# yisol/IDM-VTON

Hardware: NVIDIA H100
Metric: try-on images/sec @768x1024, 30 steps, CFG 2.0 (higher is better)
Workload: dtype fp16

## Files before the change

idm-vton_b200/csrc/attn.cu:

```cuda
#include <cuda_fp8.h>

#include <algorithm>

#include "common.cuh"
#include "host.h"
#include "wgmma.cuh"

namespace vton {

struct FlashParams {
  __half* out;
  int ld_out;
  int B, H, Nq, N0, N1;
  int D;
  int kv1_off;
  int kv1_count;
  const int* kv1_base;
  const int* kv1_rows;
  int causal;
  float scale_log2;
  int accumulate;
  float out_scale;
};

constexpr int FA_REGION = 128 * 128;
constexpr int FA_THREADS = 384;
constexpr int FA_PRODUCER_REGS = 40;
constexpr int FA_CONSUMER_REGS = 232;
constexpr uint32_t FA_BAR_TURN = 1;
constexpr uint32_t FA_BAR_CVT = 3;
constexpr int FA_CVT_THREADS = 96;

template <int R, bool KV8 = false>
struct FlashSmem {
  static constexpr int STAGES = R == 1 ? 3 : 2;
  static constexpr int OFF_Q = 0;
  static constexpr int OFF_K = OFF_Q + R * FA_REGION;
  static constexpr int OFF_V = OFF_K + STAGES * R * FA_REGION;
  static constexpr int STG_Q = 128 * 64;
  static constexpr int STG_BYTES = KV8 ? 2 * STG_Q + 2 * 128 : 0;
  static constexpr int OFF_STG = OFF_V + STAGES * R * FA_REGION;
  static constexpr int OFF_BAR = OFF_STG + STAGES * STG_BYTES;
  static constexpr int TOTAL = OFF_BAR + (KV8 ? 128 : 64) + 1024;
};

__device__ __forceinline__ float fast_exp2(float x) {
  float y;
  asm("ex2.approx.ftz.f32 %0, %1;" : "=f"(y) : "f"(x));
  return y;
}

__device__ __forceinline__ uint32_t kv8_scale_h2(int e) {
  const uint32_t hb = e >= -14 ? static_cast<uint32_t>(e + 15) << 10 : 1u << (e + 24);
  return hb | (hb << 16);
}
__device__ __forceinline__ uint32_t kv8_dequant2(uint32_t codes, uint32_t scale_h2) {
  const __half2_raw r = __nv_cvt_fp8x2_to_halfraw2(static_cast<__nv_fp8x2_storage_t>(codes & 0xffffu), __NV_E4M3);
  __half2 v(r);
  const __half2 s = *reinterpret_cast<const __half2*>(&scale_h2);
  v = __hmul2_rn(v, s);
  return *reinterpret_cast<uint32_t*>(&v);
}

template <int KS, bool IP, int R, int DN, bool KV8>
__device__ __forceinline__ void flash_body(const CUtensorMap* tmQ, const CUtensorMap* tmK0, const CUtensorMap* tmV0,
                                           const CUtensorMap* tmK1, const CUtensorMap* tmV1, const CUtensorMap* tmE,
                                           const FlashParams p) {
  static_assert(!KV8 || (KS == 4 && !IP && R == 1 && DN == 64), "the FP8 segment 1 is for D = 64 without IP");
  using SM = FlashSmem<R, KV8>;
  constexpr int ST = SM::STAGES;
  constexpr bool OVERLAP = DN == 64 && !IP;
  extern __shared__ uint8_t smem_raw[];
  const uint32_t smem_base = (smem_u32(smem_raw) + 1023u) & ~1023u;
  const uint32_t bar_base = smem_base + SM::OFF_BAR;
  const uint32_t q_full = bar_base;
  auto kv_full = [&](int s) { return bar_base + 8u * (1 + s); };
  auto kv_empty = [&](int s) { return bar_base + 8u * (1 + ST + s); };
  auto stg_full = [&](int s) { return bar_base + 8u * (1 + 2 * ST + s); };

  const int warp = threadIdx.x >> 5;
  const int lane = threadIdx.x & 31;
  const int wg = threadIdx.x >> 7;
  const int q_tile = blockIdx.x;
  const int h = blockIdx.y;
  int b = blockIdx.z;
  if (p.N1 > 0 && p.kv1_off > 0 && p.kv1_off < p.B) {
    b += p.kv1_off;
    if (b >= p.B) b -= p.B;
  }

  if (threadIdx.x == 0) {
    mbar_init(q_full, 1);
    for (int s = 0; s < ST; ++s) {
      mbar_init(kv_full(s), 1);
      mbar_init(kv_empty(s), 2);
      if constexpr (KV8) mbar_init(stg_full(s), 1);
    }
    fence_barrier_init();
  }
  if (threadIdx.x == 256) {
    tma_prefetch_desc(tmQ);
    tma_prefetch_desc(tmK0);
    tma_prefetch_desc(tmV0);
    if (p.N1 > 0) {
      tma_prefetch_desc(tmK1);
      tma_prefetch_desc(tmV1);
      if constexpr (KV8) tma_prefetch_desc(tmE);
    }
  }
  pdl_wait();
  __syncthreads();
  pdl_launch_dependents();

  const int tiles0 = (p.N0 + 127) >> 7;
  int idx1 = -1;
  if (p.N1 > 0) {
    idx1 = b - p.kv1_off;
    if (idx1 >= 0 && p.kv1_rows) {
      idx1 = p.kv1_rows[idx1];
      if (idx1 >= p.kv1_count) idx1 = -1;
    } else if (idx1 >= 0) {
      idx1 = idx1 % p.kv1_count + (p.kv1_base ? *p.kv1_base : 0);
    }
  }
  const bool zero_kv = (p.N1 > 0) && (idx1 < 0);
  const int tiles1 = (p.N1 > 0 && idx1 >= 0) ? ((p.N1 + 127) >> 7) : 0;
  const int total = p.causal ? min(tiles0, q_tile + 1) : tiles0 + tiles1;

  if (wg == 2) {
    setmaxnreg_dec<FA_PRODUCER_REGS>();
    if (threadIdx.x == 256) {
      mbar_expect_tx(q_full, R * FA_REGION);
#pragma unroll
      for (int r = 0; r < R; ++r)
        tma_load_3d(smem_base + SM::OFF_Q + r * FA_REGION, tmQ, q_full, h * p.D + r * 64, q_tile * 128, b);
      for (int j = 0; j < total; ++j) {
        const int stage = j % ST;
        if (j >= ST) mbar_wait(kv_empty(stage), ((j / ST) - 1) & 1);
        if constexpr (KV8) {
          if (j >= tiles0) {
            const uint32_t stg = smem_base + SM::OFF_STG + stage * SM::STG_BYTES;
            const int key0 = (j - tiles0) * 128;
            mbar_expect_tx(stg_full(stage), SM::STG_BYTES);
            tma_load_3d(stg, tmK1, stg_full(stage), h * 64, key0, idx1);
            tma_load_3d(stg + SM::STG_Q, tmV1, stg_full(stage), h * 64, key0, idx1);
            tma_load_3d(stg + 2 * SM::STG_Q, tmE, stg_full(stage), key0, h, idx1);
            tma_load_3d(stg + 2 * SM::STG_Q + 128, tmE, stg_full(stage), key0, p.H + h, idx1);
            continue;
          }
        }
        mbar_expect_tx(kv_full(stage), 2 * R * FA_REGION);
#pragma unroll
        for (int r = 0; r < R; ++r) {
          const uint32_t kdst = smem_base + SM::OFF_K + (stage * R + r) * FA_REGION;
          const uint32_t vdst = smem_base + SM::OFF_V + (stage * R + r) * FA_REGION;
          const int col = h * p.D + r * 64;
          if (j < tiles0) {
            tma_load_3d(kdst, tmK0, kv_full(stage), col, j * 128, b);
            tma_load_3d(vdst, tmV0, kv_full(stage), col, j * 128, b);
          } else {
            tma_load_3d(kdst, tmK1, kv_full(stage), col, (j - tiles0) * 128, idx1);
            tma_load_3d(vdst, tmV1, kv_full(stage), col, (j - tiles0) * 128, idx1);
          }
        }
      }
    } else if constexpr (KV8) {
      if (warp >= 9) {
        const int t = threadIdx.x - 288;
        for (int j = tiles0; j < total; ++j) {
          const int stage = j % ST;
          mbar_wait(stg_full(stage), ((j - tiles0) / ST) & 1);
          const uint32_t stg = smem_base + SM::OFF_STG + stage * SM::STG_BYTES;
#pragma unroll 1
          for (int c = t; c < 2 * 128 * 8; c += FA_CVT_THREADS) {
            const int kv = c >> 10, r = (c >> 3) & 127, ch = c & 7;
            uint32_t lo, hi;
            int e;
            asm volatile("ld.shared.v2.u32 {%0, %1}, [%2];" : "=r"(lo), "=r"(hi) : "r"(stg + kv * SM::STG_Q + r * 64 + ch * 8));
            asm volatile("ld.shared.s8 %0, [%1];" : "=r"(e) : "r"(stg + 2 * SM::STG_Q + kv * 128 + r));
            const uint32_t sc = kv8_scale_h2(e);
            const uint32_t dst = smem_base + (kv ? SM::OFF_V : SM::OFF_K) + stage * FA_REGION + r * 128 + ((ch ^ (r & 7)) << 4);
            asm volatile("st.shared.v4.u32 [%0], {%1, %2, %3, %4};" ::"r"(dst), "r"(kv8_dequant2(lo, sc)),
                         "r"(kv8_dequant2(lo >> 16, sc)), "r"(kv8_dequant2(hi, sc)), "r"(kv8_dequant2(hi >> 16, sc))
                         : "memory");
          }
          fence_proxy_async_smem();
          named_bar_sync(FA_BAR_CVT, FA_CVT_THREADS);
          if (t == 0) mbar_arrive(kv_full(stage));
        }
      }
    }
    return;
  }

  setmaxnreg_inc<FA_CONSUMER_REGS>();
  const int row0 = wg * 64 + ((warp & 3) << 4) + (lane >> 2);
  const int qi0 = q_tile * 128 + row0, qi1 = qi0 + 8;
  const int cq = (lane & 3) * 2;
  const float sl2 = p.scale_log2;
  float m0 = -INFINITY, m1 = -INFINITY, l0 = 0.f, l1 = 0.f;
  float o[DN / 2];
#pragma unroll
  for (int i = 0; i < DN / 2; ++i) o[i] = 0.f;
  uint32_t o_seg0[IP ? DN / 4 : 1];
#pragma unroll
  for (int i = 0; i < (IP ? DN / 4 : 1); ++i) o_seg0[i] = 0u;
  float s[64];
  uint32_t pa[8][4];

  const uint32_t q_src = smem_base + SM::OFF_Q + wg * (64 * 128);
  auto issue_s = [&](int stage) {
    const uint32_t k_src = smem_base + SM::OFF_K + stage * R * FA_REGION;
    wgmma_fence();
#pragma unroll
    for (int k = 0; k < KS; ++k) {
      const uint32_t off = (k >> 2) * FA_REGION + (k & 3) * 32;
      WgmmaF16SS<128, 0>::mma(s, make_gmma_desc_sw128(q_src + off, 0, 1024), make_gmma_desc_sw128(k_src + off, 0, 1024),
                              k > 0 ? 1 : 0);
    }
    wgmma_commit();
  };
  auto issue_pv = [&](int stage) {
    const uint32_t v_src = smem_base + SM::OFF_V + stage * R * FA_REGION;
    wgmma_fence();
#pragma unroll
    for (int kk = 0; kk < 8; ++kk)
      WgmmaF16RS<DN>::mma(o, pa[kk], make_gmma_desc_sw128(v_src + kk * 2048, FA_REGION, 1024), 1);
    wgmma_commit();
  };
  auto turn_begin = [&]() { named_bar_sync(FA_BAR_TURN + wg, 256); };
  auto turn_end = [&](bool last) {
    if (!(last && wg == 1)) named_bar_arrive(FA_BAR_TURN + (wg ^ 1), 256);
  };
  auto softmax = [&](int j, float& alpha0, float& alpha1) {
    const int key0 = (j < tiles0) ? j * 128 : (j - tiles0) * 128;
    const int kv_valid = (j < tiles0) ? min(128, p.N0 - key0) : min(128, p.N1 - key0);
    const bool masked = p.causal || kv_valid < 128;
    float mx0 = -INFINITY, mx1 = -INFINITY;
    if (masked) {
#pragma unroll
      for (int i = 0; i < 16; ++i) {
#pragma unroll
        for (int u = 0; u < 2; ++u) {
          const int col = i * 8 + cq + u;
          bool ok = col < kv_valid;
          const bool ok0 = ok && (!p.causal || key0 + col <= qi0);
          const bool ok1 = ok && (!p.causal || key0 + col <= qi1);
          if (!ok0) s[4 * i + u] = -INFINITY;
          if (!ok1) s[4 * i + 2 + u] = -INFINITY;
          mx0 = fmaxf(mx0, s[4 * i + u]);
          mx1 = fmaxf(mx1, s[4 * i + 2 + u]);
        }
      }
    } else {
#pragma unroll
      for (int i = 0; i < 16; ++i) {
#pragma unroll
        for (int u = 0; u < 2; ++u) {
          mx0 = fmaxf(mx0, s[4 * i + u]);
          mx1 = fmaxf(mx1, s[4 * i + 2 + u]);
        }
      }
    }
    mx0 = fmaxf(mx0, __shfl_xor_sync(0xffffffffu, mx0, 1));
    mx0 = fmaxf(mx0, __shfl_xor_sync(0xffffffffu, mx0, 2));
    mx1 = fmaxf(mx1, __shfl_xor_sync(0xffffffffu, mx1, 1));
    mx1 = fmaxf(mx1, __shfl_xor_sync(0xffffffffu, mx1, 2));
    const float mn0 = fmaxf(m0, mx0), mn1 = fmaxf(m1, mx1);
    alpha0 = fast_exp2((m0 - mn0) * sl2);
    alpha1 = fast_exp2((m1 - mn1) * sl2);
    const float ms0 = mn0 * sl2, ms1 = mn1 * sl2;
    m0 = mn0;
    m1 = mn1;
    float sum0 = 0.f, sum1 = 0.f;
    if (masked) {
#pragma unroll
      for (int i = 0; i < 16; ++i) {
#pragma unroll
        for (int u = 0; u < 2; ++u) {
          const float x0 = s[4 * i + u], x1 = s[4 * i + 2 + u];
          const float p0 = x0 == -INFINITY ? 0.f : fast_exp2(x0 * sl2 - ms0);
          const float p1 = x1 == -INFINITY ? 0.f : fast_exp2(x1 * sl2 - ms1);
          s[4 * i + u] = p0;
          s[4 * i + 2 + u] = p1;
          sum0 += p0;
          sum1 += p1;
        }
      }
    } else {
#pragma unroll
      for (int i = 0; i < 16; ++i) {
#pragma unroll
        for (int u = 0; u < 2; ++u) {
          const float p0 = fast_exp2(s[4 * i + u] * sl2 - ms0);
          const float p1 = fast_exp2(s[4 * i + 2 + u] * sl2 - ms1);
          s[4 * i + u] = p0;
          s[4 * i + 2 + u] = p1;
          sum0 += p0;
          sum1 += p1;
        }
      }
    }
    l0 = l0 * alpha0 + sum0;
    l1 = l1 * alpha1 + sum1;
  };
  auto pack_p = [&]() {
#pragma unroll
    for (int kk = 0; kk < 8; ++kk) {
      pa[kk][0] = pack_h2(s[8 * kk + 0], s[8 * kk + 1]);
      pa[kk][1] = pack_h2(s[8 * kk + 2], s[8 * kk + 3]);
      pa[kk][2] = pack_h2(s[8 * kk + 4], s[8 * kk + 5]);
      pa[kk][3] = pack_h2(s[8 * kk + 6], s[8 * kk + 7]);
    }
  };

  auto rescale_o = [&](float alpha0, float alpha1) {
#pragma unroll
    for (int i = 0; i < DN / 8; ++i) {
      o[4 * i] *= alpha0;
      o[4 * i + 1] *= alpha0;
      o[4 * i + 2] *= alpha1;
      o[4 * i + 3] *= alpha1;
    }
  };
  auto close_segment0 = [&](float ls0, float ls1) {
    ls0 += __shfl_xor_sync(0xffffffffu, ls0, 1);
    ls0 += __shfl_xor_sync(0xffffffffu, ls0, 2);
    ls1 += __shfl_xor_sync(0xffffffffu, ls1, 1);
    ls1 += __shfl_xor_sync(0xffffffffu, ls1, 2);
    const float i0 = 1.f / ls0, i1 = 1.f / ls1;
#pragma unroll
    for (int i = 0; i < DN / 8; ++i) {
      if constexpr (IP) {
        o_seg0[2 * i] = pack_h2(o[4 * i] * i0, o[4 * i + 1] * i0);
        o_seg0[2 * i + 1] = pack_h2(o[4 * i + 2] * i1, o[4 * i + 3] * i1);
      }
      o[4 * i] = o[4 * i + 1] = o[4 * i + 2] = o[4 * i + 3] = 0.f;
    }
  };

  if (wg == 1) named_bar_arrive(FA_BAR_TURN, 256);
  mbar_wait(q_full, 0);
  if constexpr (OVERLAP) {
    mbar_wait(kv_full(0), 0);
    turn_begin();
    issue_s(0);
    turn_end(false);
    wgmma_wait<0>();
    fence_regs(s);
    {
      float a0, a1;
      softmax(0, a0, a1);
    }
    pack_p();
    for (int j = 1; j < total; ++j) {
      const int stage = j % ST, prev = (j - 1) % ST;
      mbar_wait(kv_full(stage), (j / ST) & 1);
      turn_begin();
      issue_s(stage);
      issue_pv(prev);
      turn_end(false);
      wgmma_wait<1>();
      fence_regs(s);
      const bool seg_start = IP && j == tiles0;
      float ls0 = l0, ls1 = l1;
      if (seg_start) {
        m0 = m1 = -INFINITY;
        l0 = l1 = 0.f;
      }
      float alpha0, alpha1;
      softmax(j, alpha0, alpha1);
      wgmma_wait<0>();
      fence_regs(o);
      if ((threadIdx.x & 127) == 0) mbar_arrive(kv_empty(prev));
      if (seg_start)
        close_segment0(ls0, ls1);
      else
        rescale_o(alpha0, alpha1);
      pack_p();
    }
    turn_begin();
    issue_pv((total - 1) % ST);
    turn_end(true);
    wgmma_wait<0>();
    fence_regs(o);
  } else {
    for (int j = 0; j < total; ++j) {
      const int stage = j % ST;
      mbar_wait(kv_full(stage), (j / ST) & 1);
      turn_begin();
      issue_s(stage);
      turn_end(false);
      wgmma_wait<0>();
      fence_regs(s);
      const bool seg_start = IP && j == tiles0;
      float ls0 = l0, ls1 = l1;
      if (seg_start) {
        m0 = m1 = -INFINITY;
        l0 = l1 = 0.f;
      }
      float alpha0, alpha1;
      softmax(j, alpha0, alpha1);
      if (seg_start)
        close_segment0(ls0, ls1);
      else
        rescale_o(alpha0, alpha1);
      pack_p();
      fence_regs(o);
      turn_begin();
      issue_pv(stage);
      turn_end(j == total - 1);
      wgmma_wait<0>();
      fence_regs(o);
      if ((threadIdx.x & 127) == 0) mbar_arrive(kv_empty(stage));
    }
  }

  l0 += __shfl_xor_sync(0xffffffffu, l0, 1);
  l0 += __shfl_xor_sync(0xffffffffu, l0, 2);
  l1 += __shfl_xor_sync(0xffffffffu, l1, 1);
  l1 += __shfl_xor_sync(0xffffffffu, l1, 2);
  if (zero_kv) {
    const float mn0 = fmaxf(m0, 0.f), mn1 = fmaxf(m1, 0.f);
    const float alpha0 = fast_exp2((m0 - mn0) * sl2), alpha1 = fast_exp2((m1 - mn1) * sl2);
    l0 = l0 * alpha0 + static_cast<float>(p.N1) * fast_exp2(-mn0 * sl2);
    l1 = l1 * alpha1 + static_cast<float>(p.N1) * fast_exp2(-mn1 * sl2);
#pragma unroll
    for (int i = 0; i < DN / 8; ++i) {
      o[4 * i] *= alpha0;
      o[4 * i + 1] *= alpha0;
      o[4 * i + 2] *= alpha1;
      o[4 * i + 3] *= alpha1;
    }
  }
  const float inv[2] = {1.f / l0, 1.f / l1};
  const int qi[2] = {qi0, qi1};
  const bool two_softmax = IP && tiles1 > 0;
#pragma unroll
  for (int hr = 0; hr < 2; ++hr) {
    if (qi[hr] >= p.Nq) continue;
    __half* dst = p.out + (static_cast<long long>(b) * p.Nq + qi[hr]) * p.ld_out + h * p.D;
#pragma unroll
    for (int i = 0; i < DN / 8; ++i) {
      const int col = i * 8 + cq;
      if (col >= p.D) continue;
      float v0 = o[4 * i + 2 * hr] * inv[hr], v1 = o[4 * i + 2 * hr + 1] * inv[hr];
      if (two_softmax) {
        const float2 t = unpack_h2(o_seg0[IP ? 2 * i + hr : 0]);
        v0 = t.x + round_h(p.out_scale * round_h(v0));
        v1 = t.y + round_h(p.out_scale * round_h(v1));
      } else if (p.accumulate) {
        const float2 a = unpack_h2(*reinterpret_cast<const uint32_t*>(dst + col));
        v0 = a.x + round_h(p.out_scale * round_h(v0));
        v1 = a.y + round_h(p.out_scale * round_h(v1));
      }
      *reinterpret_cast<uint32_t*>(dst + col) = pack_h2(v0, v1);
    }
  }
}

template <int KS, bool IP = false, int R = (KS + 3) / 4, int DN = (KS <= 4 ? 64 : 96)>
__global__ void __launch_bounds__(FA_THREADS, 1)
flash_kernel(const __grid_constant__ CUtensorMap tmQ, const __grid_constant__ CUtensorMap tmK0,
             const __grid_constant__ CUtensorMap tmV0, const __grid_constant__ CUtensorMap tmK1,
             const __grid_constant__ CUtensorMap tmV1, const FlashParams p) {
  flash_body<KS, IP, R, DN, false>(&tmQ, &tmK0, &tmV0, &tmK1, &tmV1, nullptr, p);
}

__global__ void __launch_bounds__(FA_THREADS, 1)
flash_kv8_kernel(const __grid_constant__ CUtensorMap tmQ, const __grid_constant__ CUtensorMap tmK0,
                 const __grid_constant__ CUtensorMap tmV0, const __grid_constant__ CUtensorMap tmK1,
                 const __grid_constant__ CUtensorMap tmV1, const __grid_constant__ CUtensorMap tmE, const FlashParams p) {
  flash_body<4, false, 1, 64, true>(&tmQ, &tmK0, &tmV0, &tmK1, &tmV1, &tmE, p);
}

void set_attn_poly(int) {}
void set_attn_qtiles(int) {}
void set_attn_v2(int) {}

static int encode_tokens(CUtensorMap* tm, const void* base, long long ld, int cols, int n, int batch) {
  uint64_t dims[3] = {static_cast<uint64_t>(cols), static_cast<uint64_t>(n), static_cast<uint64_t>(batch)};
  uint64_t strides[2] = {static_cast<uint64_t>(ld) * 2, static_cast<uint64_t>(n) * ld * 2};
  uint32_t box[3] = {64, 128, 1};
  return encode_tmap_f16(tm, base, 3, dims, strides, box);
}

template <int KS, bool IP = false>
static int launch_flash(const CUtensorMap& tmQ, const CUtensorMap& tmK0, const CUtensorMap& tmV0, const CUtensorMap& tmK1,
                        const CUtensorMap& tmV1, const FlashParams& p, cudaStream_t stream) {
  constexpr int R = (KS + 3) / 4;
  auto kern = flash_kernel<KS, IP>;
  static bool configured = false;
  if (!configured) {
    VTON_CUDA(cudaFuncSetAttribute(kern, cudaFuncAttributeMaxDynamicSharedMemorySize, FlashSmem<R>::TOTAL));
    configured = true;
  }
  dim3 grid((p.Nq + 127) / 128, p.H, p.B);
  VTON_CUDA(launch_kernel(kern, grid, dim3(FA_THREADS), FlashSmem<R>::TOTAL, stream, tmQ, tmK0, tmV0, tmK1, tmV1, p));
  count_launch();
  return kOk;
}

static int flash(const void* q, long long ldq, const void* k0, const void* v0, long long ldkv0, const void* k1,
                 const void* v1, long long ldkv1, int B1, void* out, long long ldo, FlashParams p, cudaStream_t stream,
                 bool ip = false) {
  CUtensorMap tmQ, tmK0, tmV0, tmK1, tmV1;
  const int cols = p.H * p.D;
  if (int e = encode_tokens(&tmQ, q, ldq, cols, p.Nq, p.B)) return e;
  if (int e = encode_tokens(&tmK0, k0, ldkv0, cols, p.N0, p.B)) return e;
  if (int e = encode_tokens(&tmV0, v0, ldkv0, cols, p.N0, p.B)) return e;
  tmK1 = tmK0;
  tmV1 = tmV0;
  if (k1 != nullptr) {
    if (int e = encode_tokens(&tmK1, k1, ldkv1, cols, p.N1, B1)) return e;
    if (int e = encode_tokens(&tmV1, v1, ldkv1, cols, p.N1, B1)) return e;
  }
  p.out = static_cast<__half*>(out);
  p.ld_out = static_cast<int>(ldo);
  if (ip) return launch_flash<4, true>(tmQ, tmK0, tmV0, tmK1, tmV1, p, stream);
  switch (p.D / 16) {
    case 1: return launch_flash<1>(tmQ, tmK0, tmV0, tmK1, tmV1, p, stream);
    case 2: return launch_flash<2>(tmQ, tmK0, tmV0, tmK1, tmV1, p, stream);
    case 3: return launch_flash<3>(tmQ, tmK0, tmV0, tmK1, tmV1, p, stream);
    case 4: return launch_flash<4>(tmQ, tmK0, tmV0, tmK1, tmV1, p, stream);
    case 5: return launch_flash<5>(tmQ, tmK0, tmV0, tmK1, tmV1, p, stream);
    case 6: return launch_flash<6>(tmQ, tmK0, tmV0, tmK1, tmV1, p, stream);
  }
  set_last_error("attention: head dim %d unsupported", p.D);
  return kErrUnsupported;
}

static int attn_common(const void* q, long long ldq, const void* k0, const void* v0, long long ldkv0, const void* k1,
                       const void* v1, long long ldkv1, void* out, long long ldo, int B, int H, int Nq, int N0, int N1,
                       int B1, int kv1_off, int kv1_mod, const void* kv1_base, const void* kv1_rows, float scale,
                       int accumulate, cudaStream_t stream) {
  VTON_CHECK_ARG(B > 0 && H > 0 && Nq > 0 && N0 > 0 && N1 >= 0, "attn: bad sizes B=%d H=%d Nq=%d N0=%d N1=%d", B, H, Nq, N0, N1);
  VTON_CHECK_ARG(ldq % 8 == 0 && ldkv0 % 8 == 0 && ldo % 8 == 0, "attn: row strides must be multiples of 8");
  VTON_CHECK_ARG(aligned_to(out, 4), "attn: out must be 4-byte aligned (stored two halves at a time)");
  VTON_CHECK_ARG(B <= 65535 && H <= 65535, "attn: grid too large");
  const bool has1 = N1 > 0 && B1 > 0 && k1 && v1;
  VTON_CHECK_ARG(N1 == 0 || has1 || kv1_off >= B, "attn: segment 1 declared (N1=%d) but no K/V given", N1);
  VTON_CHECK_ARG(!has1 || ldkv1 % 8 == 0, "attn: ldkv1 must be a multiple of 8");
  FlashParams p{};
  p.B = B;
  p.H = H;
  p.Nq = Nq;
  p.N0 = N0;
  p.N1 = N1;
  p.D = 64;
  p.kv1_off = has1 ? kv1_off : (N1 > 0 ? B : 0);
  p.kv1_count = has1 ? (kv1_rows || kv1_mod <= 0 ? B1 : kv1_mod) : 1;
  p.kv1_base = has1 && !kv1_rows ? static_cast<const int*>(kv1_base) : nullptr;
  p.kv1_rows = has1 ? static_cast<const int*>(kv1_rows) : nullptr;
  p.scale_log2 = scale * 1.4426950408889634f;
  p.accumulate = accumulate;
  p.out_scale = 1.f;
  return flash(q, ldq, k0, v0, ldkv0, has1 ? k1 : nullptr, has1 ? v1 : nullptr, ldkv1, B1, out, ldo, p, stream);
}

int attn_impl(const void* q, long long ldq, const void* k0, const void* v0, long long ldkv0, const void* k1,
              const void* v1, long long ldkv1, void* out, long long ldo, int B, int H, int Nq, int N0, int N1, int B1,
              int kv1_off, int kv1_mod, const void* kv1_base, float scale, int accumulate, cudaStream_t stream) {
  return attn_common(q, ldq, k0, v0, ldkv0, k1, v1, ldkv1, out, ldo, B, H, Nq, N0, N1, B1, kv1_off, kv1_mod, kv1_base,
                     nullptr, scale, accumulate, stream);
}

int attn_rows_impl(const void* q, long long ldq, const void* k0, const void* v0, long long ldkv0, const void* k1,
                   const void* v1, long long ldkv1, void* out, long long ldo, int B, int H, int Nq, int N0, int N1,
                   int B1, int kv1_off, const void* kv1_rows, float scale, int accumulate, cudaStream_t stream) {
  VTON_CHECK_ARG(kv1_rows, "attention_rows: kv1_rows is null");
  VTON_CHECK_ARG(aligned_to(kv1_rows, 4), "attention_rows: kv1_rows must be 4-byte aligned (int32)");
  VTON_CHECK_ARG(N1 > 0 && B1 > 0 && k1 && v1, "attention_rows: needs segment-1 K/V (N1=%d, B1=%d)", N1, B1);
  VTON_CHECK_ARG(kv1_off >= 0 && kv1_off < B, "attention_rows: kv1_off %d outside [0, B=%d)", kv1_off, B);
  return attn_common(q, ldq, k0, v0, ldkv0, k1, v1, ldkv1, out, ldo, B, H, Nq, N0, N1, B1, kv1_off, 0, nullptr,
                     kv1_rows, scale, accumulate, stream);
}

int cross_attn_impl(const void* q, long long ldq, const void* kt, const void* vt, long long ldkv_t, int Nt,
                    const void* ki, const void* vi, long long ldkv_i, int Ni, void* out, long long ldo, int B, int H,
                    int Nq, float scale, float ip_scale, cudaStream_t stream) {
  VTON_CHECK_ARG(B > 0 && H > 0 && Nq > 0, "cross_attn: bad sizes B=%d H=%d Nq=%d", B, H, Nq);
  VTON_CHECK_ARG(Nt > 0 && Nt <= 80 && Ni >= 0 && Ni <= 16, "cross_attn: needs 1 <= Nt <= 80 and Ni <= 16 (got %d, %d)", Nt, Ni);
  VTON_CHECK_ARG(q && kt && vt && out && (Ni == 0 || (ki && vi)), "cross_attn: null pointer");
  VTON_CHECK_ARG(ldq % 8 == 0 && ldkv_t % 8 == 0 && ldo % 8 == 0 && (Ni == 0 || ldkv_i % 8 == 0),
                 "cross_attn: row strides must be multiples of 8");
  VTON_CHECK_ARG(aligned_to(out, 4), "cross_attn: out must be 4-byte aligned (stored two halves at a time)");
  VTON_CHECK_ARG(B <= 65535 && H <= 65535, "cross_attn: grid too large");
  FlashParams p{};
  p.B = B;
  p.H = H;
  p.Nq = Nq;
  p.N0 = Nt;
  p.N1 = Ni;
  p.D = 64;
  p.kv1_count = B;
  p.scale_log2 = scale * 1.4426950408889634f;
  p.out_scale = Ni > 0 ? ip_scale : 1.f;
  return flash(q, ldq, kt, vt, ldkv_t, Ni > 0 ? ki : nullptr, Ni > 0 ? vi : nullptr, ldkv_i, B, out, ldo, p, stream,
               Ni > 0);
}

int attn_kv8_impl(const void* q, long long ldq, const void* k0, const void* v0, long long ldkv0, const void* k1,
                  const void* v1, long long ldkv1, const void* e1, long long lde1, void* out, long long ldo, int B, int H,
                  int Nq, int N0, int N1, int B1, int kv1_off, int kv1_mod, const void* kv1_base, const void* kv1_rows,
                  float scale, int accumulate, cudaStream_t stream) {
  VTON_CHECK_ARG(B > 0 && H > 0 && Nq > 0 && N0 > 0 && N1 > 0 && B1 > 0,
                 "attention_kv8: bad sizes B=%d H=%d Nq=%d N0=%d N1=%d B1=%d", B, H, Nq, N0, N1, B1);
  VTON_CHECK_ARG(q && k0 && v0 && k1 && v1 && e1 && out, "attention_kv8: null pointer");
  VTON_CHECK_ARG(ldq % 8 == 0 && ldkv0 % 8 == 0 && ldo % 8 == 0, "attention_kv8: fp16 row strides must be multiples of 8");
  VTON_CHECK_ARG(ldkv1 % 16 == 0 && ldkv1 >= 64LL * H, "attention_kv8: ldkv1 %lld must be a multiple of 16 and >= 64*H",
                 ldkv1);
  VTON_CHECK_ARG(lde1 % 16 == 0 && lde1 >= N1, "attention_kv8: lde1 %lld must be a multiple of 16 and >= N1 = %d", lde1,
                 N1);
  VTON_CHECK_ARG(aligned_to(out, 4), "attention_kv8: out must be 4-byte aligned (stored two halves at a time)");
  VTON_CHECK_ARG(aligned_to(kv1_rows, 4), "attention_kv8: kv1_rows must be 4-byte aligned (int32)");
  VTON_CHECK_ARG(kv1_off >= 0 && kv1_off < B, "attention_kv8: kv1_off %d outside [0, B=%d)", kv1_off, B);
  VTON_CHECK_ARG(B <= 65535 && H <= 65535, "attention_kv8: grid too large");
  FlashParams p{};
  p.B = B;
  p.H = H;
  p.Nq = Nq;
  p.N0 = N0;
  p.N1 = N1;
  p.D = 64;
  p.kv1_off = kv1_off;
  p.kv1_count = kv1_rows || kv1_mod <= 0 ? B1 : kv1_mod;
  p.kv1_base = kv1_rows ? nullptr : static_cast<const int*>(kv1_base);
  p.kv1_rows = static_cast<const int*>(kv1_rows);
  p.scale_log2 = scale * 1.4426950408889634f;
  p.accumulate = accumulate;
  p.out_scale = 1.f;
  p.out = static_cast<__half*>(out);
  p.ld_out = static_cast<int>(ldo);
  CUtensorMap tmQ, tmK0, tmV0, tmK1, tmV1, tmE;
  const int cols = H * 64;
  if (int e = encode_tokens(&tmQ, q, ldq, cols, Nq, B)) return e;
  if (int e = encode_tokens(&tmK0, k0, ldkv0, cols, N0, B)) return e;
  if (int e = encode_tokens(&tmV0, v0, ldkv0, cols, N0, B)) return e;
  {
    const uint64_t dims[3] = {static_cast<uint64_t>(cols), static_cast<uint64_t>(N1), static_cast<uint64_t>(B1)};
    const uint64_t strides[2] = {static_cast<uint64_t>(ldkv1), static_cast<uint64_t>(ldkv1) * N1};
    const uint32_t box[3] = {64, 128, 1};
    if (int e = encode_tmap_u8(&tmK1, k1, 3, dims, strides, box, 0)) return e;
    if (int e = encode_tmap_u8(&tmV1, v1, 3, dims, strides, box, 0)) return e;
  }
  {
    const uint64_t dims[3] = {static_cast<uint64_t>(lde1), static_cast<uint64_t>(2 * H), static_cast<uint64_t>(B1)};
    const uint64_t strides[2] = {static_cast<uint64_t>(lde1), static_cast<uint64_t>(lde1) * 2 * H};
    const uint32_t box[3] = {128, 1, 1};
    if (int e = encode_tmap_u8(&tmE, e1, 3, dims, strides, box, 0)) return e;
  }
  using SM = FlashSmem<1, true>;
  static bool configured = false;
  if (!configured) {
    VTON_CUDA(cudaFuncSetAttribute(flash_kv8_kernel, cudaFuncAttributeMaxDynamicSharedMemorySize, SM::TOTAL));
    configured = true;
  }
  dim3 grid((Nq + 127) / 128, H, B);
  VTON_CUDA(launch_kernel(flash_kv8_kernel, grid, dim3(FA_THREADS), SM::TOTAL, stream, tmQ, tmK0, tmV0, tmK1, tmV1, tmE, p));
  count_launch();
  return kOk;
}

__global__ void __launch_bounds__(256) quantize_kv_e4m3_kernel(const __half* __restrict__ x, long long ldx, int rows,
                                                                int Ng, int G, int lde, uint8_t* __restrict__ q,
                                                                long long ldq, int8_t* __restrict__ e_out) {
  pdl_wait();
  pdl_launch_dependents();
  const int lane = threadIdx.x & 31, sub = lane & 7;
  const long long n_items = static_cast<long long>(rows) * G * lde;
  const long long warps = static_cast<long long>(gridDim.x) * (blockDim.x >> 5);
  for (long long base = (static_cast<long long>(blockIdx.x) * (blockDim.x >> 5) + (threadIdx.x >> 5)) * 4;
       base < n_items; base += warps * 4) {
    const long long it = base + (lane >> 3);
    const bool valid = it < n_items;
    const int n = valid ? static_cast<int>(it % lde) : 0;
    const long long rg = valid ? it / lde : 0;
    const int g = static_cast<int>(rg % G);
    const bool tok = valid && n < Ng;
    const long long m = (rg / G) * Ng + n;
    float v[8];
    float amax = 0.f;
    if (tok) {
      const uint4 raw = *reinterpret_cast<const uint4*>(x + m * ldx + g * 64 + sub * 8);
      const uint32_t w[4] = {raw.x, raw.y, raw.z, raw.w};
#pragma unroll
      for (int i = 0; i < 4; ++i) {
        const float2 f = unpack_h2(w[i]);
        v[2 * i] = f.x;
        v[2 * i + 1] = f.y;
        amax = fmaxf(amax, fmaxf(fabsf(f.x), fabsf(f.y)));
      }
    }
    amax = fmaxf(amax, __shfl_xor_sync(0xffffffffu, amax, 1));
    amax = fmaxf(amax, __shfl_xor_sync(0xffffffffu, amax, 2));
    amax = fmaxf(amax, __shfl_xor_sync(0xffffffffu, amax, 4));
    int e = 0;
    if (amax > 0.f) {
      const uint32_t bits = __float_as_uint(amax);
      const int E = static_cast<int>((bits >> 23) & 0xff) - 127;
      e = max(E - ((bits & 0x7fffffu) <= 0x600000u ? 8 : 7), -24);
    }
    if (tok) {
      const float inv = __uint_as_float(static_cast<uint32_t>(127 - e) << 23);
      uint32_t packed[2];
#pragma unroll
      for (int i = 0; i < 2; ++i) {
        const __nv_fp8x2_storage_t a =
            __nv_cvt_float2_to_fp8x2(make_float2(__fmul_rn(v[4 * i], inv), __fmul_rn(v[4 * i + 1], inv)), __NV_SATFINITE, __NV_E4M3);
        const __nv_fp8x2_storage_t b =
            __nv_cvt_float2_to_fp8x2(make_float2(__fmul_rn(v[4 * i + 2], inv), __fmul_rn(v[4 * i + 3], inv)), __NV_SATFINITE, __NV_E4M3);
        packed[i] = static_cast<uint32_t>(a) | (static_cast<uint32_t>(b) << 16);
      }
      *reinterpret_cast<uint2*>(q + m * ldq + g * 64 + sub * 8) = make_uint2(packed[0], packed[1]);
    }
    if (valid && sub == 0) e_out[rg * lde + n] = static_cast<int8_t>(tok ? e : 0);
  }
}

int quantize_kv_e4m3_impl(const void* x, long long ldx, int M, int G, int Ng, void* q, long long ldq, void* e,
                          long long lde, cudaStream_t stream) {
  VTON_CHECK_ARG(M > 0 && G > 0 && Ng > 0 && M % Ng == 0, "quantize_kv_e4m3: bad sizes M=%d G=%d Ng=%d (M must be a "
                 "multiple of Ng)", M, G, Ng);
  VTON_CHECK_ARG(x && q && e, "quantize_kv_e4m3: null pointer");
  VTON_CHECK_ARG(ldx % 8 == 0 && ldx >= 64LL * G && aligned_to(x, 16),
                 "quantize_kv_e4m3: x must be 16-byte aligned with ldx a multiple of 8 and >= 64*G");
  VTON_CHECK_ARG(ldq % 8 == 0 && ldq >= 64LL * G && aligned_to(q, 8),
                 "quantize_kv_e4m3: q must be 8-byte aligned with ldq a multiple of 8 and >= 64*G");
  VTON_CHECK_ARG(lde >= Ng && lde <= (1LL << 30), "quantize_kv_e4m3: lde %lld must be >= Ng = %d", lde, Ng);
  const int rows = M / Ng;
  const long long items = static_cast<long long>(rows) * G * lde;
  const long long blocks = std::min<long long>((items + 31) / 32, 32LL * num_sms());
  VTON_CUDA(launch_kernel(quantize_kv_e4m3_kernel, dim3(static_cast<unsigned>(blocks)), dim3(256), 0, stream,
                          static_cast<const __half*>(x), ldx, rows, Ng, G, static_cast<int>(lde),
                          static_cast<uint8_t*>(q), ldq, static_cast<int8_t*>(e)));
  count_launch();
  return kOk;
}

int enc_attn_impl(const void* q, long long ldq, const void* k, const void* v, long long ldkv, void* out, long long ldo,
                  int B, int H, int N, int D, float scale, int causal, cudaStream_t stream) {
  VTON_CHECK_ARG(B > 0 && H > 0 && N > 0, "encoder_attention: bad sizes B=%d H=%d N=%d", B, H, N);
  VTON_CHECK_ARG(D >= 16 && D <= 96 && D % 16 == 0, "encoder_attention: head dim %d unsupported (16..96, multiple of 16)", D);
  VTON_CHECK_ARG(ldq % 8 == 0 && ldkv % 8 == 0 && ldo % 8 == 0, "encoder_attention: row strides must be multiples of 8");
  VTON_CHECK_ARG(aligned_to(out, 4), "encoder_attention: out must be 4-byte aligned (stored two halves at a time)");
  VTON_CHECK_ARG(B <= 65535 && H <= 65535, "encoder_attention: grid too large");
  FlashParams p{};
  p.B = B;
  p.H = H;
  p.Nq = N;
  p.N0 = N;
  p.D = D;
  p.kv1_count = 1;
  p.causal = causal ? 1 : 0;
  p.scale_log2 = scale * 1.4426950408889634f;
  p.out_scale = 1.f;
  return flash(q, ldq, k, v, ldkv, nullptr, nullptr, 0, 0, out, ldo, p, stream);
}

}
```

idm-vton_b200/csrc/common.cuh:

```cuda
#pragma once
#include <cuda.h>
#include <cuda_fp16.h>
#include <cuda_runtime.h>
#include <stdint.h>
#include <stdio.h>

namespace vton {


__device__ __forceinline__ uint32_t smem_u32(const void* p) {
  return static_cast<uint32_t>(__cvta_generic_to_shared(p));
}

__device__ __forceinline__ uint64_t globaltimer_ns() {
  uint64_t t;
  asm volatile("mov.u64 %0, %globaltimer;" : "=l"(t));
  return t;
}

__device__ __forceinline__ void mbar_init(uint32_t bar, uint32_t count) {
  asm volatile("mbarrier.init.shared::cta.b64 [%0], %1;" ::"r"(bar), "r"(count) : "memory");
}
__device__ __forceinline__ void fence_barrier_init() {
  asm volatile("fence.mbarrier_init.release.cluster;" ::: "memory");
}
__device__ __forceinline__ void mbar_expect_tx(uint32_t bar, uint32_t bytes) {
  asm volatile("mbarrier.arrive.expect_tx.shared::cta.b64 _, [%0], %1;" ::"r"(bar), "r"(bytes) : "memory");
}
__device__ __forceinline__ void mbar_arrive(uint32_t bar) {
  asm volatile("mbarrier.arrive.shared::cta.b64 _, [%0];" ::"r"(bar) : "memory");
}
__device__ __forceinline__ bool mbar_try_wait(uint32_t bar, uint32_t parity) {
  uint32_t ok;
  asm volatile(
      "{\n\t.reg .pred p;\n\t"
      "mbarrier.try_wait.parity.shared::cta.b64 p, [%1], %2;\n\t"
      "selp.u32 %0, 1, 0, p;\n\t}"
      : "=r"(ok)
      : "r"(bar), "r"(parity)
      : "memory");
  return ok != 0;
}
__device__ __forceinline__ void mbar_wait(uint32_t bar, uint32_t parity) {
  if (mbar_try_wait(bar, parity)) return;
  const uint64_t t0 = globaltimer_ns();
  uint32_t spins = 0;
  while (!mbar_try_wait(bar, parity)) {
    if ((++spins & 0x3ff) == 0 && globaltimer_ns() - t0 > 4000000000ull) __trap();
  }
}

__device__ __forceinline__ void fence_proxy_async_smem() {
  asm volatile("fence.proxy.async.shared::cta;" ::: "memory");
}

__device__ __forceinline__ bool elect_one() {
  uint32_t pred;
  asm volatile(
      "{\n\t.reg .pred p;\n\t"
      "elect.sync _|p, 0xffffffff;\n\t"
      "selp.u32 %0, 1, 0, p;\n\t}"
      : "=r"(pred));
  return pred != 0;
}

__device__ __forceinline__ void tma_prefetch_desc(const CUtensorMap* m) {
  asm volatile("prefetch.tensormap [%0];" ::"l"(reinterpret_cast<uint64_t>(m)) : "memory");
}
__device__ __forceinline__ void tma_load_2d(uint32_t dst, const CUtensorMap* m, uint32_t bar, int c0, int c1) {
  asm volatile(
      "cp.async.bulk.tensor.2d.shared::cluster.global.mbarrier::complete_tx::bytes [%0], [%1, {%3, %4}], [%2];"
      ::"r"(dst), "l"(reinterpret_cast<uint64_t>(m)), "r"(bar), "r"(c0), "r"(c1)
      : "memory");
}
__device__ __forceinline__ void tma_load_3d(uint32_t dst, const CUtensorMap* m, uint32_t bar, int c0, int c1,
                                            int c2) {
  asm volatile(
      "cp.async.bulk.tensor.3d.shared::cluster.global.mbarrier::complete_tx::bytes [%0], [%1, {%3, %4, %5}], [%2];"
      ::"r"(dst), "l"(reinterpret_cast<uint64_t>(m)), "r"(bar), "r"(c0), "r"(c1), "r"(c2)
      : "memory");
}
__device__ __forceinline__ void tma_load_4d(uint32_t dst, const CUtensorMap* m, uint32_t bar, int c0, int c1,
                                            int c2, int c3) {
  asm volatile(
      "cp.async.bulk.tensor.4d.shared::cluster.global.mbarrier::complete_tx::bytes [%0], [%1, {%3, %4, %5, %6}], "
      "[%2];"
      ::"r"(dst), "l"(reinterpret_cast<uint64_t>(m)), "r"(bar), "r"(c0), "r"(c1), "r"(c2), "r"(c3)
      : "memory");
}

__device__ __forceinline__ void pdl_launch_dependents() { asm volatile("griddepcontrol.launch_dependents;" ::: "memory"); }
__device__ __forceinline__ void pdl_wait() { asm volatile("griddepcontrol.wait;" ::: "memory"); }

__device__ __forceinline__ void wgmma_fence() { asm volatile("wgmma.fence.sync.aligned;" ::: "memory"); }
__device__ __forceinline__ void wgmma_commit() { asm volatile("wgmma.commit_group.sync.aligned;" ::: "memory"); }
template <int N>
__device__ __forceinline__ void wgmma_wait() {
  asm volatile("wgmma.wait_group.sync.aligned %0;" ::"n"(N) : "memory");
}
template <int N>
__device__ __forceinline__ void fence_regs(float (&r)[N]) {
#pragma unroll
  for (int i = 0; i < N; ++i) asm volatile("" : "+f"(r[i])::"memory");
}

__device__ __forceinline__ uint64_t make_gmma_desc_sw128(uint32_t saddr, uint32_t lbo_bytes, uint32_t sbo_bytes) {
  uint64_t d = 0;
  d |= static_cast<uint64_t>((saddr & 0x3ffff) >> 4);
  d |= static_cast<uint64_t>((lbo_bytes >> 4) & 0x3fff) << 16;
  d |= static_cast<uint64_t>((sbo_bytes >> 4) & 0x3fff) << 32;
  d |= static_cast<uint64_t>(1) << 62;
  return d;
}

__device__ __forceinline__ void named_bar_sync(uint32_t id, uint32_t nthreads) {
  asm volatile("bar.sync %0, %1;" ::"r"(id), "r"(nthreads) : "memory");
}
__device__ __forceinline__ void named_bar_arrive(uint32_t id, uint32_t nthreads) {
  asm volatile("bar.arrive %0, %1;" ::"r"(id), "r"(nthreads) : "memory");
}

template <int N>
__device__ __forceinline__ void setmaxnreg_dec() { asm volatile("setmaxnreg.dec.sync.aligned.u32 %0;" ::"n"(N)); }
template <int N>
__device__ __forceinline__ void setmaxnreg_inc() { asm volatile("setmaxnreg.inc.sync.aligned.u32 %0;" ::"n"(N)); }

__device__ __forceinline__ float h2f(__half h) { return __half2float(h); }
__device__ __forceinline__ __half f2h(float f) { return __float2half_rn(f); }
__device__ __forceinline__ float round_h(float f) { return __half2float(__float2half_rn(f)); }
__device__ __forceinline__ float silu_f(float x) { return x / (1.0f + __expf(-x)); }
__device__ __forceinline__ float gelu_erf_f(float x) { return 0.5f * x * (1.0f + erff(x * 0.70710678118654752f)); }
__device__ __forceinline__ uint32_t pack_h2(float a, float b) {
  __half2 h = __floats2half2_rn(a, b);
  return *reinterpret_cast<uint32_t*>(&h);
}
__device__ __forceinline__ float2 unpack_h2(uint32_t u) {
  __half2 h = *reinterpret_cast<__half2*>(&u);
  return __half22float2(h);
}

}
```

Baseline: 0.9212.

## Make self-attention flash kernel persistent with multi-slot Q prefetch and TMA output stores

Adds a persistent variant of the flash attention kernel for the plain self-attention path (no second KV segment, no IP). It launches one CTA per SM that loops over (q_tile, head, batch) items, with Q multi-buffered across items and a continuous K/V ring counter. Output now goes through shared memory and a TMA tensor store, which lets the epilogue of one item overlap the next item's loads. The aim is to remove per-CTA launch, barrier-init and tail costs. In exchange it adds shared-memory pressure, a static round-robin schedule that may balance poorly, and more complex phase tracking.

```diff
diff --git a/idm-vton_b200/csrc/attn.cu b/idm-vton_b200/csrc/attn.cu
--- a/idm-vton_b200/csrc/attn.cu
+++ b/idm-vton_b200/csrc/attn.cu
@@ -21,6 +21,7 @@
   float scale_log2;
   int accumulate;
   float out_scale;
+  int out_col;
 };
 
 constexpr int FA_REGION = 128 * 128;
@@ -29,90 +30,32 @@
 constexpr int FA_CONSUMER_REGS = 232;
 constexpr uint32_t FA_BAR_TURN = 1;
 constexpr uint32_t FA_BAR_CVT = 3;
+constexpr uint32_t FA_BAR_EPI = 4;
 constexpr int FA_CVT_THREADS = 96;
 
-template <int R, bool KV8 = false>
-struct FlashSmem {
-  static constexpr int STAGES = R == 1 ? 3 : 2;
-  static constexpr int OFF_Q = 0;
-  static constexpr int OFF_K = OFF_Q + R * FA_REGION;
-  static constexpr int OFF_V = OFF_K + STAGES * R * FA_REGION;
-  static constexpr int STG_Q = 128 * 64;
-  static constexpr int STG_BYTES = KV8 ? 2 * STG_Q + 2 * 128 : 0;
-  static constexpr int OFF_STG = OFF_V + STAGES * R * FA_REGION;
-  static constexpr int OFF_BAR = OFF_STG + STAGES * STG_BYTES;
-  static constexpr int TOTAL = OFF_BAR + (KV8 ? 128 : 64) + 1024;
+struct FlashItem {
+  int b, h, q_tile, idx1, tiles0, tiles1, total;
 };
-
-__device__ __forceinline__ float fast_exp2(float x) {
-  float y;
-  asm("ex2.approx.ftz.f32 %0, %1;" : "=f"(y) : "f"(x));
-  return y;
-}
-
-__device__ __forceinline__ uint32_t kv8_scale_h2(int e) {
-  const uint32_t hb = e >= -14 ? static_cast<uint32_t>(e + 15) << 10 : 1u << (e + 24);
-  return hb | (hb << 16);
-}
-__device__ __forceinline__ uint32_t kv8_dequant2(uint32_t codes, uint32_t scale_h2) {
-  const __half2_raw r = __nv_cvt_fp8x2_to_halfraw2(static_cast<__nv_fp8x2_storage_t>(codes & 0xffffu), __NV_E4M3);
-  __half2 v(r);
-  const __half2 s = *reinterpret_cast<const __half2*>(&scale_h2);
-  v = __hmul2_rn(v, s);
-  return *reinterpret_cast<uint32_t*>(&v);
-}
-
-template <int KS, bool IP, int R, int DN, bool KV8>
-__device__ __forceinline__ void flash_body(const CUtensorMap* tmQ, const CUtensorMap* tmK0, const CUtensorMap* tmV0,
-                                           const CUtensorMap* tmK1, const CUtensorMap* tmV1, const CUtensorMap* tmE,
-                                           const FlashParams p) {
-  static_assert(!KV8 || (KS == 4 && !IP && R == 1 && DN == 64), "the FP8 segment 1 is for D = 64 without IP");
-  using SM = FlashSmem<R, KV8>;
-  constexpr int ST = SM::STAGES;
-  constexpr bool OVERLAP = DN == 64 && !IP;
-  extern __shared__ uint8_t smem_raw[];
-  const uint32_t smem_base = (smem_u32(smem_raw) + 1023u) & ~1023u;
-  const uint32_t bar_base = smem_base + SM::OFF_BAR;
-  const uint32_t q_full = bar_base;
-  auto kv_full = [&](int s) { return bar_base + 8u * (1 + s); };
-  auto kv_empty = [&](int s) { return bar_base + 8u * (1 + ST + s); };
-  auto stg_full = [&](int s) { return bar_base + 8u * (1 + 2 * ST + s); };
-
-  const int warp = threadIdx.x >> 5;
-  const int lane = threadIdx.x & 31;
-  const int wg = threadIdx.x >> 7;
-  const int q_tile = blockIdx.x;
-  const int h = blockIdx.y;
-  int b = blockIdx.z;
+template <bool PERSIST>
+__device__ __forceinline__ FlashItem flash_item(const FlashParams& p, int item) {
+  FlashItem t;
+  int b;
+  if constexpr (PERSIST) {
+    const int qt = (p.Nq + 127) >> 7;
+    t.q_tile = item % qt;
+    t.h = (item / qt) % p.H;
+    b = item / qt / p.H;
+  } else {
+    t.q_tile = blockIdx.x;
+    t.h = blockIdx.y;
+    b = blockIdx.z;
+  }
   if (p.N1 > 0 && p.kv1_off > 0 && p.kv1_off < p.B) {
     b += p.kv1_off;
     if (b >= p.B) b -= p.B;
   }
-
-  if (threadIdx.x == 0) {
-    mbar_init(q_full, 1);
-    for (int s = 0; s < ST; ++s) {
-      mbar_init(kv_full(s), 1);
-      mbar_init(kv_empty(s), 2);
-      if constexpr (KV8) mbar_init(stg_full(s), 1);
-    }
-    fence_barrier_init();
-  }
-  if (threadIdx.x == 256) {
-    tma_prefetch_desc(tmQ);
-    tma_prefetch_desc(tmK0);
-    tma_prefetch_desc(tmV0);
-    if (p.N1 > 0) {
-      tma_prefetch_desc(tmK1);
-      tma_prefetch_desc(tmV1);
-      if constexpr (KV8) tma_prefetch_desc(tmE);
-    }
-  }
-  pdl_wait();
-  __syncthreads();
-  pdl_launch_dependents();
-
-  const int tiles0 = (p.N0 + 127) >> 7;
+  t.b = b;
+  t.tiles0 = (p.N0 + 127) >> 7;
   int idx1 = -1;
   if (p.N1 > 0) {
     idx1 = b - p.kv1_off;
@@ -123,70 +66,173 @@
       idx1 = idx1 % p.kv1_count + (p.kv1_base ? *p.kv1_base : 0);
     }
   }
-  const bool zero_kv = (p.N1 > 0) && (idx1 < 0);
-  const int tiles1 = (p.N1 > 0 && idx1 >= 0) ? ((p.N1 + 127) >> 7) : 0;
-  const int total = p.causal ? min(tiles0, q_tile + 1) : tiles0 + tiles1;
+  t.idx1 = idx1;
+  t.tiles1 = (p.N1 > 0 && idx1 >= 0) ? ((p.N1 + 127) >> 7) : 0;
+  t.total = p.causal ? min(t.tiles0, t.q_tile + 1) : t.tiles0 + t.tiles1;
+  return t;
+}
+
+template <int R, bool KV8, bool PERSIST>
+struct FlashSmem {
+  static constexpr int STAGES = R == 1 ? 3 : 2;
+  static constexpr int Q_SLOTS = !PERSIST ? 1 : R == 1 ? 4 : 2;
+  static constexpr int OFF_Q = 0;
+  static constexpr int OFF_K = OFF_Q + Q_SLOTS * R * FA_REGION;
+  static constexpr int OFF_V = OFF_K + STAGES * R * FA_REGION;
+  static constexpr int STG_Q = 128 * 64;
+  static constexpr int STG_BYTES = KV8 ? 2 * STG_Q + 2 * 128 : 0;
+  static constexpr int OFF_STG = OFF_V + STAGES * R * FA_REGION;
+  static constexpr int O_WG = PERSIST ? 64 * (R == 1 ? 64 : 96) * 2 : 0;
+  static constexpr int OFF_O = (OFF_STG + STAGES * STG_BYTES + 1023) & ~1023;
+  static constexpr int OFF_BAR = OFF_O + 2 * O_WG;
+  static constexpr int TOTAL = OFF_BAR + 8 * (2 * Q_SLOTS + 3 * STAGES) + 1024;
+  static_assert(TOTAL <= 227 * 1024, "shared memory");
+};
+
+__device__ __forceinline__ float fast_exp2(float x) {
+  float y;
+  asm("ex2.approx.ftz.f32 %0, %1;" : "=f"(y) : "f"(x));
+  return y;
+}
+
+__device__ __forceinline__ uint32_t kv8_scale_h2(int e) {
+  const uint32_t hb = e >= -14 ? static_cast<uint32_t>(e + 15) << 10 : 1u << (e + 24);
+  return hb | (hb << 16);
+}
+__device__ __forceinline__ uint32_t kv8_dequant2(uint32_t codes, uint32_t scale_h2) {
+  const __half2_raw r = __nv_cvt_fp8x2_to_halfraw2(static_cast<__nv_fp8x2_storage_t>(codes & 0xffffu), __NV_E4M3);
+  __half2 v(r);
+  const __half2 s = *reinterpret_cast<const __half2*>(&scale_h2);
+  v = __hmul2_rn(v, s);
+  return *reinterpret_cast<uint32_t*>(&v);
+}
+
+template <int KS, bool IP, int R, int DN, bool KV8, bool PERSIST>
+__device__ __forceinline__ void flash_body(const CUtensorMap* tmQ, const CUtensorMap* tmK0, const CUtensorMap* tmV0,
+                                           const CUtensorMap* tmK1, const CUtensorMap* tmV1, const CUtensorMap* tmE,
+                                           const CUtensorMap* tmO, const FlashParams p) {
+  static_assert(!KV8 || (KS == 4 && !IP && R == 1 && DN == 64), "the FP8 segment 1 is for D = 64 without IP");
+  using SM = FlashSmem<R, KV8, PERSIST>;
+  constexpr int ST = SM::STAGES;
+  constexpr int QS = SM::Q_SLOTS;
+  constexpr bool OVERLAP = DN == 64 && !IP;
+  extern __shared__ uint8_t smem_raw[];
+  const uint32_t smem_base = (smem_u32(smem_raw) + 1023u) & ~1023u;
+  const uint32_t bar_base = smem_base + SM::OFF_BAR;
+  auto q_full = [&](int s) { return bar_base + 8u * s; };
+  auto q_empty = [&](int s) { return bar_base + 8u * (QS + s); };
+  auto kv_full = [&](int s) { return bar_base + 8u * (2 * QS + s); };
+  auto kv_empty = [&](int s) { return bar_base + 8u * (2 * QS + ST + s); };
+  auto stg_full = [&](int s) { return bar_base + 8u * (2 * QS + 2 * ST + s); };
+
+  const int warp = threadIdx.x >> 5;
+  const int lane = threadIdx.x & 31;
+  const int wg = threadIdx.x >> 7;
+  const int n_items = PERSIST ? ((p.Nq + 127) >> 7) * p.H * p.B : 1;
+  const int first_item = PERSIST ? static_cast<int>(blockIdx.x) : 0;
+
+  if (threadIdx.x == 0) {
+    for (int s = 0; s < QS; ++s) {
+      mbar_init(q_full(s), 1);
+      mbar_init(q_empty(s), 2);
+    }
+    for (int s = 0; s < ST; ++s) {
+      mbar_init(kv_full(s), 1);
+      mbar_init(kv_empty(s), 2);
+      if constexpr (KV8) mbar_init(stg_full(s), 1);
+    }
+    fence_barrier_init();
+  }
+  if (threadIdx.x == 256) {
+    tma_prefetch_desc(tmQ);
+    tma_prefetch_desc(tmK0);
+    tma_prefetch_desc(tmV0);
+    if constexpr (PERSIST) tma_prefetch_desc(tmO);
+    if (p.N1 > 0) {
+      tma_prefetch_desc(tmK1);
+      tma_prefetch_desc(tmV1);
+      if constexpr (KV8) tma_prefetch_desc(tmE);
+    }
+  }
+  pdl_wait();
+  __syncthreads();
+  pdl_launch_dependents();
 
   if (wg == 2) {
     setmaxnreg_dec<FA_PRODUCER_REGS>();
     if (threadIdx.x == 256) {
-      mbar_expect_tx(q_full, R * FA_REGION);
-#pragma unroll
-      for (int r = 0; r < R; ++r)
-        tma_load_3d(smem_base + SM::OFF_Q + r * FA_REGION, tmQ, q_full, h * p.D + r * 64, q_tile * 128, b);
-      for (int j = 0; j < total; ++j) {
-        const int stage = j % ST;
-        if (j >= ST) mbar_wait(kv_empty(stage), ((j / ST) - 1) & 1);
-        if constexpr (KV8) {
-          if (j >= tiles0) {
-            const uint32_t stg = smem_base + SM::OFF_STG + stage * SM::STG_BYTES;
-            const int key0 = (j - tiles0) * 128;
-            mbar_expect_tx(stg_full(stage), SM::STG_BYTES);
-            tma_load_3d(stg, tmK1, stg_full(stage), h * 64, key0, idx1);
-            tma_load_3d(stg + SM::STG_Q, tmV1, stg_full(stage), h * 64, key0, idx1);
-            tma_load_3d(stg + 2 * SM::STG_Q, tmE, stg_full(stage), key0, h, idx1);
-            tma_load_3d(stg + 2 * SM::STG_Q + 128, tmE, stg_full(stage), key0, p.H + h, idx1);
-            continue;
+      int it = 0;
+      for (int n = 0, item = first_item; item < n_items; item += gridDim.x, ++n) {
+        const FlashItem t = flash_item<PERSIST>(p, item);
+        const int slot = n % QS;
+        if (n >= QS) mbar_wait(q_empty(slot), ((n / QS) - 1) & 1);
+        mbar_expect_tx(q_full(slot), R * FA_REGION);
+#pragma unroll
+        for (int r = 0; r < R; ++r)
+          tma_load_3d(smem_base + SM::OFF_Q + (slot * R + r) * FA_REGION, tmQ, q_full(slot), t.h * p.D + r * 64,
+                      t.q_tile * 128, t.b);
+        for (int j = 0; j < t.total; ++j, ++it) {
+          const int stage = it % ST;
+          if (it >= ST) mbar_wait(kv_empty(stage), ((it / ST) - 1) & 1);
+          if constexpr (KV8) {
+            if (j >= t.tiles0) {
+              const uint32_t stg = smem_base + SM::OFF_STG + stage * SM::STG_BYTES;
+              const int key0 = (j - t.tiles0) * 128;
+              mbar_expect_tx(stg_full(stage), SM::STG_BYTES);
+              tma_load_3d(stg, tmK1, stg_full(stage), t.h * 64, key0, t.idx1);
+              tma_load_3d(stg + SM::STG_Q, tmV1, stg_full(stage), t.h * 64, key0, t.idx1);
+              tma_load_3d(stg + 2 * SM::STG_Q, tmE, stg_full(stage), key0, t.h, t.idx1);
+              tma_load_3d(stg + 2 * SM::STG_Q + 128, tmE, stg_full(stage), key0, p.H + t.h, t.idx1);
+              continue;
+            }
+          }
+          mbar_expect_tx(kv_full(stage), 2 * R * FA_REGION);
+#pragma unroll
+          for (int r = 0; r < R; ++r) {
+            const uint32_t kdst = smem_base + SM::OFF_K + (stage * R + r) * FA_REGION;
+            const uint32_t vdst = smem_base + SM::OFF_V + (stage * R + r) * FA_REGION;
+            const int col = t.h * p.D + r * 64;
+            if (j < t.tiles0) {
+              tma_load_3d(kdst, tmK0, kv_full(stage), col, j * 128, t.b);
+              tma_load_3d(vdst, tmV0, kv_full(stage), col, j * 128, t.b);
+            } else {
+              tma_load_3d(kdst, tmK1, kv_full(stage), col, (j - t.tiles0) * 128, t.idx1);
+              tma_load_3d(vdst, tmV1, kv_full(stage), col, (j - t.tiles0) * 128, t.idx1);
+            }
           }
         }
-        mbar_expect_tx(kv_full(stage), 2 * R * FA_REGION);
-#pragma unroll
-        for (int r = 0; r < R; ++r) {
-          const uint32_t kdst = smem_base + SM::OFF_K + (stage * R + r) * FA_REGION;
-          const uint32_t vdst = smem_base + SM::OFF_V + (stage * R + r) * FA_REGION;
-          const int col = h * p.D + r * 64;
-          if (j < tiles0) {
-            tma_load_3d(kdst, tmK0, kv_full(stage), col, j * 128, b);
-            tma_load_3d(vdst, tmV0, kv_full(stage), col, j * 128, b);
-          } else {
-            tma_load_3d(kdst, tmK1, kv_full(stage), col, (j - tiles0) * 128, idx1);
-            tma_load_3d(vdst, tmV1, kv_full(stage), col, (j - tiles0) * 128, idx1);
-          }
-        }
+        if constexpr (!PERSIST) break;
       }
     } else if constexpr (KV8) {
       if (warp >= 9) {
         const int t = threadIdx.x - 288;
-        for (int j = tiles0; j < total; ++j) {
-          const int stage = j % ST;
-          mbar_wait(stg_full(stage), ((j - tiles0) / ST) & 1);
-          const uint32_t stg = smem_base + SM::OFF_STG + stage * SM::STG_BYTES;
+        int it = 0;
+        uint32_t stg_phase = 0;
+        for (int item = first_item; item < n_items; item += gridDim.x) {
+          const FlashItem f = flash_item<PERSIST>(p, item);
+          it += f.tiles0;
+          for (int j = f.tiles0; j < f.total; ++j, ++it) {
+            const int stage = it % ST;
+            mbar_wait(stg_full(stage), (stg_phase >> stage) & 1);
+            stg_phase ^= 1u << stage;
+            const uint32_t stg = smem_base + SM::OFF_STG + stage * SM::STG_BYTES;
 #pragma unroll 1
-          for (int c = t; c < 2 * 128 * 8; c += FA_CVT_THREADS) {
-            const int kv = c >> 10, r = (c >> 3) & 127, ch = c & 7;
-            uint32_t lo, hi;
-            int e;
-            asm volatile("ld.shared.v2.u32 {%0, %1}, [%2];" : "=r"(lo), "=r"(hi) : "r"(stg + kv * SM::STG_Q + r * 64 + ch * 8));
-            asm volatile("ld.shared.s8 %0, [%1];" : "=r"(e) : "r"(stg + 2 * SM::STG_Q + kv * 128 + r));
-            const uint32_t sc = kv8_scale_h2(e);
-            const uint32_t dst = smem_base + (kv ? SM::OFF_V : SM::OFF_K) + stage * FA_REGION + r * 128 + ((ch ^ (r & 7)) << 4);
-            asm volatile("st.shared.v4.u32 [%0], {%1, %2, %3, %4};" ::"r"(dst), "r"(kv8_dequant2(lo, sc)),
-                         "r"(kv8_dequant2(lo >> 16, sc)), "r"(kv8_dequant2(hi, sc)), "r"(kv8_dequant2(hi >> 16, sc))
-                         : "memory");
+            for (int c = t; c < 2 * 128 * 8; c += FA_CVT_THREADS) {
+              const int kv = c >> 10, r = (c >> 3) & 127, ch = c & 7;
+              uint32_t lo, hi;
+              int e;
+              asm volatile("ld.shared.v2.u32 {%0, %1}, [%2];" : "=r"(lo), "=r"(hi) : "r"(stg + kv * SM::STG_Q + r * 64 + ch * 8));
+              asm volatile("ld.shared.s8 %0, [%1];" : "=r"(e) : "r"(stg + 2 * SM::STG_Q + kv * 128 + r));
+              const uint32_t sc = kv8_scale_h2(e);
+              const uint32_t dst = smem_base + (kv ? SM::OFF_V : SM::OFF_K) + stage * FA_REGION + r * 128 + ((ch ^ (r & 7)) << 4);
+              asm volatile("st.shared.v4.u32 [%0], {%1, %2, %3, %4};" ::"r"(dst), "r"(kv8_dequant2(lo, sc)),
+                           "r"(kv8_dequant2(lo >> 16, sc)), "r"(kv8_dequant2(hi, sc)), "r"(kv8_dequant2(hi >> 16, sc))
+                           : "memory");
+            }
+            fence_proxy_async_smem();
+            named_bar_sync(FA_BAR_CVT, FA_CVT_THREADS);
+            if (t == 0) mbar_arrive(kv_full(stage));
           }
-          fence_proxy_async_smem();
-          named_bar_sync(FA_BAR_CVT, FA_CVT_THREADS);
-          if (t == 0) mbar_arrive(kv_full(stage));
         }
       }
     }
@@ -194,21 +240,17 @@
   }
 
   setmaxnreg_inc<FA_CONSUMER_REGS>();
-  const int row0 = wg * 64 + ((warp & 3) << 4) + (lane >> 2);
-  const int qi0 = q_tile * 128 + row0, qi1 = qi0 + 8;
+  const int row0 = ((warp & 3) << 4) + (lane >> 2);
   const int cq = (lane & 3) * 2;
   const float sl2 = p.scale_log2;
-  float m0 = -INFINITY, m1 = -INFINITY, l0 = 0.f, l1 = 0.f;
+  float m0, m1, l0, l1;
   float o[DN / 2];
-#pragma unroll
-  for (int i = 0; i < DN / 2; ++i) o[i] = 0.f;
   uint32_t o_seg0[IP ? DN / 4 : 1];
-#pragma unroll
-  for (int i = 0; i < (IP ? DN / 4 : 1); ++i) o_seg0[i] = 0u;
   float s[64];
   uint32_t pa[8][4];
-
-  const uint32_t q_src = smem_base + SM::OFF_Q + wg * (64 * 128);
+  uint32_t q_src = 0;
+  int qi0 = 0, qi1 = 0, tiles0 = 0, it = 0;
+
   auto issue_s = [&](int stage) {
     const uint32_t k_src = smem_base + SM::OFF_K + stage * R * FA_REGION;
     wgmma_fence();
@@ -339,139 +381,182 @@
     }
   };
 
+  const bool store_thread = (threadIdx.x & 127) == 0;
+  const uint32_t o_tile = smem_base + SM::OFF_O + wg * SM::O_WG;
   if (wg == 1) named_bar_arrive(FA_BAR_TURN, 256);
-  mbar_wait(q_full, 0);
-  if constexpr (OVERLAP) {
-    mbar_wait(kv_full(0), 0);
-    turn_begin();
-    issue_s(0);
-    turn_end(false);
-    wgmma_wait<0>();
-    fence_regs(s);
-    {
-      float a0, a1;
-      softmax(0, a0, a1);
-    }
-    pack_p();
-    for (int j = 1; j < total; ++j) {
-      const int stage = j % ST, prev = (j - 1) % ST;
-      mbar_wait(kv_full(stage), (j / ST) & 1);
+  for (int n = 0, item = first_item; item < n_items; item += gridDim.x, ++n) {
+    const bool last_item = !PERSIST || item + static_cast<int>(gridDim.x) >= n_items;
+    const FlashItem t = flash_item<PERSIST>(p, item);
+    const int slot = n % QS;
+    const int total = t.total;
+    tiles0 = t.tiles0;
+    q_src = smem_base + SM::OFF_Q + slot * R * FA_REGION + wg * (64 * 128);
+    qi0 = t.q_tile * 128 + wg * 64 + row0;
+    qi1 = qi0 + 8;
+    m0 = m1 = -INFINITY;
+    l0 = l1 = 0.f;
+#pragma unroll
+    for (int i = 0; i < DN / 2; ++i) o[i] = 0.f;
+#pragma unroll
+    for (int i = 0; i < (IP ? DN / 4 : 1); ++i) o_seg0[i] = 0u;
+
+    mbar_wait(q_full(slot), (n / QS) & 1);
+    if constexpr (OVERLAP) {
+      mbar_wait(kv_full(it % ST), (it / ST) & 1);
       turn_begin();
-      issue_s(stage);
-      issue_pv(prev);
-      turn_end(false);
-      wgmma_wait<1>();
-      fence_regs(s);
-      const bool seg_start = IP && j == tiles0;
-      float ls0 = l0, ls1 = l1;
-      if (seg_start) {
-        m0 = m1 = -INFINITY;
-        l0 = l1 = 0.f;
-      }
-      float alpha0, alpha1;
-      softmax(j, alpha0, alpha1);
-      wgmma_wait<0>();
-      fence_regs(o);
-      if ((threadIdx.x & 127) == 0) mbar_arrive(kv_empty(prev));
-      if (seg_start)
-        close_segment0(ls0, ls1);
-      else
-        rescale_o(alpha0, alpha1);
-      pack_p();
-    }
-    turn_begin();
-    issue_pv((total - 1) % ST);
-    turn_end(true);
-    wgmma_wait<0>();
-    fence_regs(o);
-  } else {
-    for (int j = 0; j < total; ++j) {
-      const int stage = j % ST;
-      mbar_wait(kv_full(stage), (j / ST) & 1);
-      turn_begin();
-      issue_s(stage);
+      issue_s(it % ST);
       turn_end(false);
       wgmma_wait<0>();
       fence_regs(s);
-      const bool seg_start = IP && j == tiles0;
-      float ls0 = l0, ls1 = l1;
-      if (seg_start) {
-        m0 = m1 = -INFINITY;
-        l0 = l1 = 0.f;
-      }
-      float alpha0, alpha1;
-      softmax(j, alpha0, alpha1);
-      if (seg_start)
-        close_segment0(ls0, ls1);
-      else
+      {
+        float a0, a1;
+        softmax(0, a0, a1);
+      }
+      pack_p();
+      for (int j = 1; j < total; ++j) {
+        const int stage = (it + j) % ST, prev = (it + j - 1) % ST;
+        mbar_wait(kv_full(stage), ((it + j) / ST) & 1);
+        turn_begin();
+        issue_s(stage);
+        issue_pv(prev);
+        turn_end(false);
+        wgmma_wait<1>();
+        fence_regs(s);
+        float alpha0, alpha1;
+        softmax(j, alpha0, alpha1);
+        wgmma_wait<0>();
+        fence_regs(o);
+        if (store_thread) mbar_arrive(kv_empty(prev));
         rescale_o(alpha0, alpha1);
-      pack_p();
-      fence_regs(o);
+        pack_p();
+      }
+      const int last = (it + total - 1) % ST;
       turn_begin();
-      issue_pv(stage);
-      turn_end(j == total - 1);
+      issue_pv(last);
+      turn_end(last_item);
       wgmma_wait<0>();
       fence_regs(o);
-      if ((threadIdx.x & 127) == 0) mbar_arrive(kv_empty(stage));
-    }
-  }
-
-  l0 += __shfl_xor_sync(0xffffffffu, l0, 1);
-  l0 += __shfl_xor_sync(0xffffffffu, l0, 2);
-  l1 += __shfl_xor_sync(0xffffffffu, l1, 1);
-  l1 += __shfl_xor_sync(0xffffffffu, l1, 2);
-  if (zero_kv) {
-    const float mn0 = fmaxf(m0, 0.f), mn1 = fmaxf(m1, 0.f);
-    const float alpha0 = fast_exp2((m0 - mn0) * sl2), alpha1 = fast_exp2((m1 - mn1) * sl2);
-    l0 = l0 * alpha0 + static_cast<float>(p.N1) * fast_exp2(-mn0 * sl2);
-    l1 = l1 * alpha1 + static_cast<float>(p.N1) * fast_exp2(-mn1 * sl2);
-#pragma unroll
-    for (int i = 0; i < DN / 8; ++i) {
-      o[4 * i] *= alpha0;
-      o[4 * i + 1] *= alpha0;
-      o[4 * i + 2] *= alpha1;
-      o[4 * i + 3] *= alpha1;
-    }
-  }
-  const float inv[2] = {1.f / l0, 1.f / l1};
-  const int qi[2] = {qi0, qi1};
-  const bool two_softmax = IP && tiles1 > 0;
-#pragma unroll
-  for (int hr = 0; hr < 2; ++hr) {
-    if (qi[hr] >= p.Nq) continue;
-    __half* dst = p.out + (static_cast<long long>(b) * p.Nq + qi[hr]) * p.ld_out + h * p.D;
-#pragma unroll
-    for (int i = 0; i < DN / 8; ++i) {
-      const int col = i * 8 + cq;
-      if (col >= p.D) continue;
-      float v0 = o[4 * i + 2 * hr] * inv[hr], v1 = o[4 * i + 2 * hr + 1] * inv[hr];
-      if (two_softmax) {
-        const float2 t = unpack_h2(o_seg0[IP ? 2 * i + hr : 0]);
-        v0 = t.x + round_h(p.out_scale * round_h(v0));
-        v1 = t.y + round_h(p.out_scale * round_h(v1));
-      } else if (p.accumulate) {
-        const float2 a = unpack_h2(*reinterpret_cast<const uint32_t*>(dst + col));
-        v0 = a.x + round_h(p.out_scale * round_h(v0));
-        v1 = a.y + round_h(p.out_scale * round_h(v1));
-      }
-      *reinterpret_cast<uint32_t*>(dst + col) = pack_h2(v0, v1);
-    }
-  }
-}
-
-template <int KS, bool IP = false, int R = (KS + 3) / 4, int DN = (KS <= 4 ? 64 : 96)>
+      if (store_thread) mbar_arrive(kv_empty(last));
+    } else {
+      for (int j = 0; j < total; ++j) {
+        const int stage = (it + j) % ST;
+        mbar_wait(kv_full(stage), ((it + j) / ST) & 1);
+        turn_begin();
+        issue_s(stage);
+        turn_end(false);
+        wgmma_wait<0>();
+        fence_regs(s);
+        const bool seg_start = IP && j == tiles0;
+        float ls0 = l0, ls1 = l1;
+        if (seg_start) {
+          m0 = m1 = -INFINITY;
+          l0 = l1 = 0.f;
+        }
+        float alpha0, alpha1;
+        softmax(j, alpha0, alpha1);
+        if (seg_start)
+          close_segment0(ls0, ls1);
+        else
+          rescale_o(alpha0, alpha1);
+        pack_p();
+        fence_regs(o);
+        turn_begin();
+        issue_pv(stage);
+        turn_end(j == total - 1 && last_item);
+        wgmma_wait<0>();
+        fence_regs(o);
+        if (store_thread) mbar_arrive(kv_empty(stage));
+      }
+    }
+    it += total;
+    if (store_thread) mbar_arrive(q_empty(slot));
+
+    l0 += __shfl_xor_sync(0xffffffffu, l0, 1);
+    l0 += __shfl_xor_sync(0xffffffffu, l0, 2);
+    l1 += __shfl_xor_sync(0xffffffffu, l1, 1);
+    l1 += __shfl_xor_sync(0xffffffffu, l1, 2);
+    if (t.idx1 < 0 && p.N1 > 0) {
+      const float mn0 = fmaxf(m0, 0.f), mn1 = fmaxf(m1, 0.f);
+      const float alpha0 = fast_exp2((m0 - mn0) * sl2), alpha1 = fast_exp2((m1 - mn1) * sl2);
+      l0 = l0 * alpha0 + static_cast<float>(p.N1) * fast_exp2(-mn0 * sl2);
+      l1 = l1 * alpha1 + static_cast<float>(p.N1) * fast_exp2(-mn1 * sl2);
+      rescale_o(alpha0, alpha1);
+    }
+    const float inv[2] = {1.f / l0, 1.f / l1};
+    const bool two_softmax = IP && t.tiles1 > 0;
+    if (!PERSIST || p.accumulate) {
+      const int qi[2] = {qi0, qi1};
+#pragma unroll
+      for (int hr = 0; hr < 2; ++hr) {
+        if (qi[hr] >= p.Nq) continue;
+        __half* dst = p.out + (static_cast<long long>(t.b) * p.Nq + qi[hr]) * p.ld_out + t.h * p.D;
+#pragma unroll
+        for (int i = 0; i < DN / 8; ++i) {
+          const int col = i * 8 + cq;
+          if (col >= p.D) continue;
+          float v0 = o[4 * i + 2 * hr] * inv[hr], v1 = o[4 * i + 2 * hr + 1] * inv[hr];
+          if (two_softmax) {
+            const float2 u = unpack_h2(o_seg0[IP ? 2 * i + hr : 0]);
+            v0 = u.x + round_h(p.out_scale * round_h(v0));
+            v1 = u.y + round_h(p.out_scale * round_h(v1));
+          } else if (p.accumulate) {
+            const float2 a = unpack_h2(*reinterpret_cast<const uint32_t*>(dst + col));
+            v0 = a.x + round_h(p.out_scale * round_h(v0));
+            v1 = a.y + round_h(p.out_scale * round_h(v1));
+          }
+          *reinterpret_cast<uint32_t*>(dst + col) = pack_h2(v0, v1);
+        }
+      }
+      if constexpr (!PERSIST) break;
+      continue;
+    }
+    if constexpr (PERSIST) {
+      if (store_thread) bulk_wait_read();
+      named_bar_sync(FA_BAR_EPI + wg, 128);
+#pragma unroll
+      for (int hr = 0; hr < 2; ++hr) {
+#pragma unroll
+        for (int i = 0; i < DN / 8; ++i) {
+          const int col = i * 8 + cq;
+          if (col >= p.D) continue;
+          float v0 = o[4 * i + 2 * hr] * inv[hr], v1 = o[4 * i + 2 * hr + 1] * inv[hr];
+          if (two_softmax) {
+            const float2 u = unpack_h2(o_seg0[IP ? 2 * i + hr : 0]);
+            v0 = u.x + round_h(p.out_scale * round_h(v0));
+            v1 = u.y + round_h(p.out_scale * round_h(v1));
+          }
+          const int r = row0 + 8 * hr;
+          const uint32_t dst = o_tile + (p.D == 64 ? r * 128 + (((i ^ (r & 7)) << 4) | (cq * 2)) : (r * p.D + col) * 2);
+          asm volatile("st.shared.u32 [%0], %1;" ::"r"(dst), "r"(pack_h2(v0, v1)) : "memory");
+        }
+      }
+      fence_proxy_async_smem();
+      named_bar_sync(FA_BAR_EPI + wg, 128);
+      if (store_thread) {
+        tma_store_3d(tmO, o_tile, p.out_col + t.h * p.D, t.q_tile * 128 + wg * 64, t.b);
+        bulk_commit();
+      }
+    }
+  }
+  if constexpr (PERSIST) {
+    if (store_thread) bulk_wait_read();
+  }
+}
+
+template <int KS, bool IP, bool PERSIST, int R = (KS + 3) / 4, int DN = (KS <= 4 ? 64 : 96)>
 __global__ void __launch_bounds__(FA_THREADS, 1)
 flash_kernel(const __grid_constant__ CUtensorMap tmQ, const __grid_constant__ CUtensorMap tmK0,
              const __grid_constant__ CUtensorMap tmV0, const __grid_constant__ CUtensorMap tmK1,
-             const __grid_constant__ CUtensorMap tmV1, const FlashParams p) {
-  flash_body<KS, IP, R, DN, false>(&tmQ, &tmK0, &tmV0, &tmK1, &tmV1, nullptr, p);
+             const __grid_constant__ CUtensorMap tmV1, const __grid_constant__ CUtensorMap tmO, const FlashParams p) {
+  flash_body<KS, IP, R, DN, false, PERSIST>(&tmQ, &tmK0, &tmV0, &tmK1, &tmV1, nullptr, &tmO, p);
 }
 
 __global__ void __launch_bounds__(FA_THREADS, 1)
 flash_kv8_kernel(const __grid_constant__ CUtensorMap tmQ, const __grid_constant__ CUtensorMap tmK0,
                  const __grid_constant__ CUtensorMap tmV0, const __grid_constant__ CUtensorMap tmK1,
-                 const __grid_constant__ CUtensorMap tmV1, const __grid_constant__ CUtensorMap tmE, const FlashParams p) {
-  flash_body<4, false, 1, 64, true>(&tmQ, &tmK0, &tmV0, &tmK1, &tmV1, &tmE, p);
+                 const __grid_constant__ CUtensorMap tmV1, const __grid_constant__ CUtensorMap tmE,
+                 const __grid_constant__ CUtensorMap tmO, const FlashParams p) {
+  flash_body<4, false, 1, 64, true, false>(&tmQ, &tmK0, &tmV0, &tmK1, &tmV1, &tmE, &tmO, p);
 }
 
 void set_attn_poly(int) {}
@@ -485,18 +570,43 @@
   return encode_tmap_f16(tm, base, 3, dims, strides, box);
 }
 
+static int encode_out(CUtensorMap* tm, FlashParams* p, void* out, long long ld, int cols) {
+  p->out = static_cast<__half*>(out);
+  p->ld_out = static_cast<int>(ld);
+  p->out_col = static_cast<int>((reinterpret_cast<uintptr_t>(out) & 15) / 2);
+  uint64_t dims[3] = {static_cast<uint64_t>(cols + p->out_col), static_cast<uint64_t>(p->Nq), static_cast<uint64_t>(p->B)};
+  uint64_t strides[2] = {static_cast<uint64_t>(ld) * 2, static_cast<uint64_t>(p->Nq) * ld * 2};
+  uint32_t box[3] = {static_cast<uint32_t>(p->D), 64, 1};
+  return encode_tmap_f16(tm, static_cast<__half*>(out) - p->out_col, 3, dims, strides, box, nullptr,
+                         p->D == 64 ? 128 : 0);
+}
+
 template <int KS, bool IP = false>
 static int launch_flash(const CUtensorMap& tmQ, const CUtensorMap& tmK0, const CUtensorMap& tmV0, const CUtensorMap& tmK1,
-                        const CUtensorMap& tmV1, const FlashParams& p, cudaStream_t stream) {
+                        const CUtensorMap& tmV1, const CUtensorMap& tmO, const FlashParams& p, cudaStream_t stream) {
   constexpr int R = (KS + 3) / 4;
-  auto kern = flash_kernel<KS, IP>;
-  static bool configured = false;
-  if (!configured) {
-    VTON_CUDA(cudaFuncSetAttribute(kern, cudaFuncAttributeMaxDynamicSharedMemorySize, FlashSmem<R>::TOTAL));
-    configured = true;
-  }
-  dim3 grid((p.Nq + 127) / 128, p.H, p.B);
-  VTON_CUDA(launch_kernel(kern, grid, dim3(FA_THREADS), FlashSmem<R>::TOTAL, stream, tmQ, tmK0, tmV0, tmK1, tmV1, p));
+  const long long items = static_cast<long long>((p.Nq + 127) / 128) * p.H * p.B;
+  if (p.N1 > 0 || IP) {
+    auto kern = flash_kernel<KS, IP, false>;
+    constexpr int smem = FlashSmem<R, false, false>::TOTAL;
+    static bool configured = false;
+    if (!configured) {
+      VTON_CUDA(cudaFuncSetAttribute(kern, cudaFuncAttributeMaxDynamicSharedMemorySize, smem));
+      configured = true;
+    }
+    VTON_CUDA(launch_kernel(kern, dim3((p.Nq + 127) / 128, p.H, p.B), dim3(FA_THREADS), smem, stream, tmQ, tmK0, tmV0,
+                            tmK1, tmV1, tmO, p));
+  } else {
+    auto kern = flash_kernel<KS, false, true>;
+    constexpr int smem = FlashSmem<R, false, true>::TOTAL;
+    static bool configured = false;
+    if (!configured) {
+      VTON_CUDA(cudaFuncSetAttribute(kern, cudaFuncAttributeMaxDynamicSharedMemorySize, smem));
+      configured = true;
+    }
+    VTON_CUDA(launch_kernel(kern, dim3(static_cast<unsigned>(std::min<long long>(items, num_sms()))), dim3(FA_THREADS),
+                            smem, stream, tmQ, tmK0, tmV0, tmK1, tmV1, tmO, p));
+  }
   count_launch();
   return kOk;
 }
@@ -504,7 +614,7 @@
 static int flash(const void* q, long long ldq, const void* k0, const void* v0, long long ldkv0, const void* k1,
                  const void* v1, long long ldkv1, int B1, void* out, long long ldo, FlashParams p, cudaStream_t stream,
                  bool ip = false) {
-  CUtensorMap tmQ, tmK0, tmV0, tmK1, tmV1;
+  CUtensorMap tmQ, tmK0, tmV0, tmK1, tmV1, tmO;
   const int cols = p.H * p.D;
   if (int e = encode_tokens(&tmQ, q, ldq, cols, p.Nq, p.B)) return e;
   if (int e = encode_tokens(&tmK0, k0, ldkv0, cols, p.N0, p.B)) return e;
@@ -515,16 +625,15 @@
     if (int e = encode_tokens(&tmK1, k1, ldkv1, cols, p.N1, B1)) return e;
     if (int e = encode_tokens(&tmV1, v1, ldkv1, cols, p.N1, B1)) return e;
   }
-  p.out = static_cast<__half*>(out);
-  p.ld_out = static_cast<int>(ldo);
-  if (ip) return launch_flash<4, true>(tmQ, tmK0, tmV0, tmK1, tmV1, p, stream);
+  if (int e = encode_out(&tmO, &p, out, ldo, cols)) return e;
+  if (ip) return launch_flash<4, true>(tmQ, tmK0, tmV0, tmK1, tmV1, tmO, p, stream);
   switch (p.D / 16) {
-    case 1: return launch_flash<1>(tmQ, tmK0, tmV0, tmK1, tmV1, p, stream);
-    case 2: return launch_flash<2>(tmQ, tmK0, tmV0, tmK1, tmV1, p, stream);
-    case 3: return launch_flash<3>(tmQ, tmK0, tmV0, tmK1, tmV1, p, stream);
-    case 4: return launch_flash<4>(tmQ, tmK0, tmV0, tmK1, tmV1, p, stream);
-    case 5: return launch_flash<5>(tmQ, tmK0, tmV0, tmK1, tmV1, p, stream);
-    case 6: return launch_flash<6>(tmQ, tmK0, tmV0, tmK1, tmV1, p, stream);
+    case 1: return launch_flash<1>(tmQ, tmK0, tmV0, tmK1, tmV1, tmO, p, stream);
+    case 2: return launch_flash<2>(tmQ, tmK0, tmV0, tmK1, tmV1, tmO, p, stream);
+    case 3: return launch_flash<3>(tmQ, tmK0, tmV0, tmK1, tmV1, tmO, p, stream);
+    case 4: return launch_flash<4>(tmQ, tmK0, tmV0, tmK1, tmV1, tmO, p, stream);
+    case 5: return launch_flash<5>(tmQ, tmK0, tmV0, tmK1, tmV1, tmO, p, stream);
+    case 6: return launch_flash<6>(tmQ, tmK0, tmV0, tmK1, tmV1, tmO, p, stream);
   }
   set_last_error("attention: head dim %d unsupported", p.D);
   return kErrUnsupported;
@@ -537,7 +646,7 @@
   VTON_CHECK_ARG(B > 0 && H > 0 && Nq > 0 && N0 > 0 && N1 >= 0, "attn: bad sizes B=%d H=%d Nq=%d N0=%d N1=%d", B, H, Nq, N0, N1);
   VTON_CHECK_ARG(ldq % 8 == 0 && ldkv0 % 8 == 0 && ldo % 8 == 0, "attn: row strides must be multiples of 8");
   VTON_CHECK_ARG(aligned_to(out, 4), "attn: out must be 4-byte aligned (stored two halves at a time)");
-  VTON_CHECK_ARG(B <= 65535 && H <= 65535, "attn: grid too large");
+  VTON_CHECK_ARG(B <= 65535 && H <= 65535 && 1LL * ((Nq + 127) / 128) * H * B <= INT_MAX, "attn: grid too large");
   const bool has1 = N1 > 0 && B1 > 0 && k1 && v1;
   VTON_CHECK_ARG(N1 == 0 || has1 || kv1_off >= B, "attn: segment 1 declared (N1=%d) but no K/V given", N1);
   VTON_CHECK_ARG(!has1 || ldkv1 % 8 == 0, "attn: ldkv1 must be a multiple of 8");
@@ -585,7 +694,7 @@
   VTON_CHECK_ARG(ldq % 8 == 0 && ldkv_t % 8 == 0 && ldo % 8 == 0 && (Ni == 0 || ldkv_i % 8 == 0),
                  "cross_attn: row strides must be multiples of 8");
   VTON_CHECK_ARG(aligned_to(out, 4), "cross_attn: out must be 4-byte aligned (stored two halves at a time)");
-  VTON_CHECK_ARG(B <= 65535 && H <= 65535, "cross_attn: grid too large");
+  VTON_CHECK_ARG(B <= 65535 && H <= 65535 && 1LL * ((Nq + 127) / 128) * H * B <= INT_MAX, "cross_attn: grid too large");
   FlashParams p{};
   p.B = B;
   p.H = H;
@@ -615,7 +724,7 @@
   VTON_CHECK_ARG(aligned_to(out, 4), "attention_kv8: out must be 4-byte aligned (stored two halves at a time)");
   VTON_CHECK_ARG(aligned_to(kv1_rows, 4), "attention_kv8: kv1_rows must be 4-byte aligned (int32)");
   VTON_CHECK_ARG(kv1_off >= 0 && kv1_off < B, "attention_kv8: kv1_off %d outside [0, B=%d)", kv1_off, B);
-  VTON_CHECK_ARG(B <= 65535 && H <= 65535, "attention_kv8: grid too large");
+  VTON_CHECK_ARG(B <= 65535 && H <= 65535 && 1LL * ((Nq + 127) / 128) * H * B <= INT_MAX, "attention_kv8: grid too large");
   FlashParams p{};
   p.B = B;
   p.H = H;
@@ -630,10 +739,9 @@
   p.scale_log2 = scale * 1.4426950408889634f;
   p.accumulate = accumulate;
   p.out_scale = 1.f;
-  p.out = static_cast<__half*>(out);
-  p.ld_out = static_cast<int>(ldo);
-  CUtensorMap tmQ, tmK0, tmV0, tmK1, tmV1, tmE;
+  CUtensorMap tmQ, tmK0, tmV0, tmK1, tmV1, tmE, tmO;
   const int cols = H * 64;
+  if (int e = encode_out(&tmO, &p, out, ldo, cols)) return e;
   if (int e = encode_tokens(&tmQ, q, ldq, cols, Nq, B)) return e;
   if (int e = encode_tokens(&tmK0, k0, ldkv0, cols, N0, B)) return e;
   if (int e = encode_tokens(&tmV0, v0, ldkv0, cols, N0, B)) return e;
@@ -650,14 +758,14 @@
     const uint32_t box[3] = {128, 1, 1};
     if (int e = encode_tmap_u8(&tmE, e1, 3, dims, strides, box, 0)) return e;
   }
-  using SM = FlashSmem<1, true>;
+  using SM = FlashSmem<1, true, false>;
   static bool configured = false;
   if (!configured) {
     VTON_CUDA(cudaFuncSetAttribute(flash_kv8_kernel, cudaFuncAttributeMaxDynamicSharedMemorySize, SM::TOTAL));
     configured = true;
   }
-  dim3 grid((Nq + 127) / 128, H, B);
-  VTON_CUDA(launch_kernel(flash_kv8_kernel, grid, dim3(FA_THREADS), SM::TOTAL, stream, tmQ, tmK0, tmV0, tmK1, tmV1, tmE, p));
+  VTON_CUDA(launch_kernel(flash_kv8_kernel, dim3((Nq + 127) / 128, H, B), dim3(FA_THREADS), SM::TOTAL, stream, tmQ, tmK0, tmV0,
+                          tmK1, tmV1, tmE, tmO, p));
   count_launch();
   return kOk;
 }
@@ -744,7 +852,7 @@
   VTON_CHECK_ARG(D >= 16 && D <= 96 && D % 16 == 0, "encoder_attention: head dim %d unsupported (16..96, multiple of 16)", D);
   VTON_CHECK_ARG(ldq % 8 == 0 && ldkv % 8 == 0 && ldo % 8 == 0, "encoder_attention: row strides must be multiples of 8");
   VTON_CHECK_ARG(aligned_to(out, 4), "encoder_attention: out must be 4-byte aligned (stored two halves at a time)");
-  VTON_CHECK_ARG(B <= 65535 && H <= 65535, "encoder_attention: grid too large");
+  VTON_CHECK_ARG(B <= 65535 && H <= 65535 && 1LL * ((N + 127) / 128) * H * B <= INT_MAX, "encoder_attention: grid too large");
   FlashParams p{};
   p.B = B;
   p.H = H;
diff --git a/idm-vton_b200/csrc/common.cuh b/idm-vton_b200/csrc/common.cuh
--- a/idm-vton_b200/csrc/common.cuh
+++ b/idm-vton_b200/csrc/common.cuh
@@ -89,6 +89,14 @@
       : "memory");
 }
 
+__device__ __forceinline__ void tma_store_3d(const CUtensorMap* m, uint32_t src, int c0, int c1, int c2) {
+  asm volatile("cp.async.bulk.tensor.3d.global.shared::cta.bulk_group [%0, {%2, %3, %4}], [%1];"
+               ::"l"(reinterpret_cast<uint64_t>(m)), "r"(src), "r"(c0), "r"(c1), "r"(c2)
+               : "memory");
+}
+__device__ __forceinline__ void bulk_commit() { asm volatile("cp.async.bulk.commit_group;" ::: "memory"); }
+__device__ __forceinline__ void bulk_wait_read() { asm volatile("cp.async.bulk.wait_group.read 0;" ::: "memory"); }
+
 __device__ __forceinline__ void pdl_launch_dependents() { asm volatile("griddepcontrol.launch_dependents;" ::: "memory"); }
 __device__ __forceinline__ void pdl_wait() { asm volatile("griddepcontrol.wait;" ::: "memory"); }
 
```

After: 0.9237, median of 6. Within noise of the previous version (+0.3%).
